# sair-lab/AirSLAM

Measured on AMD Instinct MI355X. Metric: stereo detect+match pairs/sec (2x PLNet @512x512 internal: points + lines, junctions on the left + LightGlue match), higher is better.
Workload: dtype fp16

## Files before the change

### airslam_amd/_lib.py

```python
from __future__ import annotations

import ctypes as C
import os

_HERE = os.path.dirname(os.path.abspath(__file__))
LIB_PATH = os.path.join(_HERE, "libairfe.so")


class Tuning(C.Structure):
    _fields_ = [(n, C.c_int) for n in (
        "fuse_lg_block", "gemm_small_max_m", "gemm8_min_m", "gemmr_min_m", "gemmr_wgs", "qkv_pair", "block_min_m", "lgb_tokens", "sg_kenc_gemm",
        "fold_qkv", "overlap_lines", "kf_graph", "kf_spec_rows", "fuse_dec", "assign_fused", "fold_out_proj", "desc_gather_stream", "copy_wgs")] + [("reserved", C.c_int * 5)]


class Cfg(C.Structure):
    _fields_ = [
        ("device", C.c_int), ("precision", C.c_int), ("max_batch", C.c_int), ("enc_chunk", C.c_int),
        ("max_keypoints", C.c_int), ("keypoint_threshold", C.c_float), ("remove_borders", C.c_int),
        ("nms_radius", C.c_int), ("line_threshold", C.c_float), ("line_length_threshold", C.c_float),
        ("matcher", C.c_int), ("image_width", C.c_int), ("image_height", C.c_int), ("sinkhorn_iters", C.c_int),
        ("superpoint_pack", C.c_char_p), ("plnet_s1_pack", C.c_char_p), ("lightglue_pack", C.c_char_p),
        ("superglue_pack", C.c_char_p), ("matcher_precision", C.c_int), ("line_precision", C.c_int), ("check_launches", C.c_int),
        ("tuning", C.POINTER(Tuning)),
    ]


class Stage0(C.Structure):
# ... 224 lines not shown
```

### airslam_amd/api.py

```python
from __future__ import annotations

import ctypes as C
import os
import tempfile
from typing import Dict, Optional

import numpy as np

from . import _lib, weights as W

FEAT = 259


def _pack_arg(x, tmpfiles) -> Optional[bytes]:
    if x is None:
        return None
    if isinstance(x, (str, bytes, os.PathLike)):
        return os.fsencode(x)
    f = tempfile.NamedTemporaryFile(suffix=".airfe", delete=False)
    f.close()
    W.save_pack(f.name, x)
    tmpfiles.append(f.name)
    return f.name.encode()

# ... 485 lines not shown
    def debug_lg_block(self, attn, x32, w1, b1, w2, b2, prec, gamma=None, beta=None, wo=None, bo=None, relu=False, tokens_per_wg=128, mixed=False,
                       nqk=None, nv=None, rot=None, Np=0):
        f32 = lambda t: None if t is None else np.ascontiguousarray(t, np.float32)
        m = attn.shape[0]
        attn, w1, b1, w2, b2, gamma, beta, wo, bo = map(f32, (attn, w1, b1, w2, b2, gamma, beta, wo, bo))
        x32 = np.array(x32, np.float32, copy=True)
        xb = np.empty_like(x32)
        ptr = lambda t: None if t is None else t.ctypes.data
        a = _lib.DebugLgBlockArgs(prec=prec, M=m, attn=ptr(attn), x32=ptr(x32), xb=ptr(xb), wo=ptr(wo), bo=ptr(bo), w1=ptr(w1), b1=ptr(b1), gamma=ptr(gamma),
                                  beta=ptr(beta), w2=ptr(w2), b2=ptr(b2), relu=int(relu), tokens_per_wg=tokens_per_wg, mixed=int(mixed), Np=Np)
        q = k = vt = None
        keep = []
        if nqk is not None:
            (qw, qb), (vw, vb) = map(lambda p: (f32(p[0]), f32(p[1])), (nqk, nv))
            keep += [qw, qb, vw, vb]
            s = m // Np
            q, vt = np.empty((s, 4, Np, 64), np.float32), np.empty((s, 4, 64, Np), np.float32)
            a.nqk_n, a.nqk_w, a.nqk_b, a.nv_w, a.nv_b, a.q, a.vt = qw.shape[0], ptr(qw), ptr(qb), ptr(vw), ptr(vb), ptr(q), ptr(vt)
            if qw.shape[0] == 512:
                k = np.empty_like(q)
                a.k = ptr(k)
        if rot is not None:
            rc, rs = f32(rot[0]), f32(rot[1])
            keep += [rc, rs]
            a.rot_cos, a.rot_sin = ptr(rc), ptr(rs)
        self._chk(self._l.airfe_debug_lg_block(self._h, C.byref(a)), "airfe_debug_lg_block")
        return {"x32": x32, "xb": xb, "q": q, "k": k, "vt": vt, "rows_past": list(a.rows_past)}

    def debug_ln_gelu(self, h, gamma, beta, prec):
        h = np.array(h, np.float32, copy=True)
        gamma, beta = np.ascontiguousarray(gamma, np.float32), np.ascontiguousarray(beta, np.float32)
# ... 476 lines not shown
```

### airslam_amd/csrc/airfe.hip

```cpp
#include "airfe_host.h"
#include "fransac_core.h"
#include "pnp_core.h"
#include "poseopt_core.h"
#include "bowgroup_core.h"

namespace airfe_host {
thread_local std::string g_err;

int fail(airfe_ctx* c, const std::string& m) {
  if (c) c->err = m;
  g_err = m;
  return 1;
}

int fail_noexcept(airfe_ctx* c, const char* what, const char* detail) noexcept {
  try {
    std::string m = std::string("airfe: C++ exception at the C boundary (") + what + "): " + (detail ? detail : "unknown");
    if (c) c->err = m;
    g_err = m;
  } catch (...) {
  }
  return 1;
}

// ... 184 lines not shown
    if (t->block_min_m >= 0) c->block_min = t->block_min_m;
    if (t->lgb_tokens >= 0) {
      if (t->lgb_tokens != 32 && t->lgb_tokens != 64 && t->lgb_tokens != 112 && t->lgb_tokens != 128) { return fail(nullptr, "airfe_create: tuning.lgb_tokens must be 32, 64, 112 or 128"); }
      c->lgb_tokens = t->lgb_tokens;
    }
    if (t->sg_kenc_gemm >= 0) c->sg_kenc_gemm = t->sg_kenc_gemm != 0;
    if (t->fold_qkv >= 0) c->fold_qkv = t->fold_qkv != 0;
    if (t->overlap_lines >= 0) c->overlap_lines = t->overlap_lines != 0;
    if (t->kf_graph >= 0) c->kf_graph_on = t->kf_graph != 0;
    if (t->kf_spec_rows >= 0) c->kf_spec_lines = c->kf_spec_juncs = std::max(t->kf_spec_rows, 1);
    if (t->fuse_dec >= 0) c->fuse_dec = t->fuse_dec != 0;
    if (t->assign_fused >= 0) c->assign_fused = t->assign_fused != 0 ? 1 : 0;
    if (t->fold_out_proj >= 0) c->fold_out = t->fold_out_proj != 0;
    if (t->desc_gather_stream >= 0) c->desc_gather_stream = t->desc_gather_stream != 0;
    if (t->copy_wgs > 0) c->copy_wgs = t->copy_wgs;
  }
  if (hipStreamCreateWithFlags(&c->stream, hipStreamNonBlocking) != hipSuccess ||
      hipStreamCreateWithFlags(&c->stream2, hipStreamNonBlocking) != hipSuccess ||
      hipEventCreateWithFlags(&c->ev_fork, hipEventDisableTiming) != hipSuccess ||
      hipEventCreateWithFlags(&c->ev_join, hipEventDisableTiming) != hipSuccess ||
      hipEventCreateWithFlags(&c->ev_feat, hipEventDisableTiming) != hipSuccess)
    return fail(nullptr, "airfe_create: stream creation failed");
  c->Dmax = (c->prec != 2 && cfg->superpoint_pack && cfg->lightglue_pack) ? 2 * c->Bmax : c->Bmax;
  c->chunk = std::min(std::max(cfg->enc_chunk, 1), c->Dmax);
  c->Lmax = c->Dmax;
  int rc = 0;
  if (cfg->superpoint_pack) rc = load_superpoint(c, cfg->superpoint_pack);
  if (!rc && cfg->lightglue_pack) rc = load_lightglue(c, cfg->lightglue_pack);
  if (!rc && cfg->superglue_pack) rc = load_superglue(c, cfg->superglue_pack);
  if (!rc && cfg->plnet_s1_pack) rc = load_plnet_s1(c, cfg->plnet_s1_pack);
// ... 1763 lines not shown
  return rc;
} AIRFE_CATCH(c)

int airfe_debug_lg_block(airfe_ctx* c, airfe_debug_lg_block_args* a) try {
  AIRFE_ENTER(c);
  if (!a || !a->attn || !a->x32 || !a->xb || !a->w1 || !a->b1 || !a->w2 || !a->b2 || (!a->relu && (!a->gamma || !a->beta)) || (!a->wo) != (!a->bo))
    return fail(c, "debug_lg_block: null argument");
  const int prec = a->prec, M = a->M, T = a->tokens_per_wg, nq = a->nqk_n, Np = a->Np;
  if ((prec != 0 && prec != 1) || M < 1 || (T != 32 && T != 64 && T != 112 && T != 128) || (nq != 0 && nq != 256 && nq != 512) || (a->relu && nq))
    return fail(c, "debug_lg_block: bad argument");
  if (a->mixed) {
    const int tiles = (M + 15) / 16, W = c->n_cu;
    if (a->wo || T != 112 || W <= 0 || tiles <= 7 * W || tiles > 13 * W) return fail(c, "debug_lg_block: the mixed split does not apply to this form");
  }
  if (nq && (!a->nqk_w || !a->nqk_b || !a->nv_w || !a->nv_b || !a->q || !a->vt || (nq == 512) != (a->rot_cos && a->rot_sin) || (nq == 512 && !a->k) || Np < 16 ||
             Np % 16 || M % Np))
    return fail(c, "debug_lg_block: the next projection needs its weights and outputs, rotary exactly when nqk_n = 512, and M = S * Np (Np a multiple of 16)");
  const int cap = M + 256;
  const int Sg = nq ? (cap + Np - 1) / Np : 0, S = nq ? M / Np : 0;
  const size_t helems = (size_t)Sg * 4 * Np * 64;
  airfe_ctx tmp;
  tmp.prec = prec;
  tmp.pack_prec = prec;
  LinW lo, l1, l2, lq, lv;
  bool ok = (!a->wo || make_linear(&tmp, a->wo, a->bo, 256, 256, lo)) && make_linear(&tmp, a->w1, a->b1, 512, 512, l1) && make_linear(&tmp, a->w2, a->b2, 512, 256, l2) &&
            (!nq || (make_linear(&tmp, a->nqk_w, a->nqk_b, 256, nq, lq) && make_linear(&tmp, a->nv_w, a->nv_b, 256, 256, lv)));
  const bool fr = lg_blockf_frag_weights();
  std::vector<float> x32h = dbg_rows4(a->x32, M, 256, cap);
  std::vector<uint16_t> xbh((size_t)cap * 256);
  for (size_t i = 0; i < xbh.size(); ++i) xbh[i] = cvt2(x32h[i], prec);
  std::vector<float> gb(1024, 0.f);
  if (!a->relu) { memcpy(gb.data(), a->gamma, 512 * 4); memcpy(gb.data() + 512, a->beta, 512 * 4); }
  LgBlockFArgs g;
  g.attn = dupload(&tmp, dbg_rows2(a->attn, M, 256, cap, prec));
  g.xb = dupload(&tmp, xbh);
  g.x32 = dupload(&tmp, x32h);
  const float* dgb = dupload(&tmp, gb);
  g.wo = a->wo ? (fr ? lo.wf : lo.w) : nullptr; g.bo = a->wo ? lo.b : nullptr;
  g.w1 = fr ? l1.wf : l1.w; g.b1 = l1.b; g.w2 = fr ? l2.wf : l2.w; g.b2 = l2.b;
  g.gamma = dgb; g.beta = dgb ? dgb + 512 : nullptr;
  g.M = M; g.tokens_per_wg = T; g.mixed = a->mixed; g.n_cu = c->n_cu; g.relu = a->relu;
  if (nq) {
    g.nqk_w = fr ? lq.wf : lq.w; g.nqk_b = lq.b; g.nqk_n = nq; g.nv_w = fr ? lv.wf : lv.w; g.nv_b = lv.b; g.Np = Np; g.H = 4;
    if (nq == 512) { g.rot_cos = dupload(&tmp, dbg_rows4(a->rot_cos, M, 32, cap)); g.rot_sin = dupload(&tmp, dbg_rows4(a->rot_sin, M, 32, cap)); }
    g.q_out = dbg_canary<uint16_t>(&tmp, helems);
    if (nq == 512) g.k_out = dbg_canary<uint16_t>(&tmp, helems);
    g.vt_out = dbg_canary<uint16_t>(&tmp, helems);
  }
  ok = ok && g.attn && g.xb && g.x32 && dgb && (!nq || (g.q_out && g.vt_out && (nq != 512 || (g.k_out && g.rot_cos && g.rot_sin))));
  int rc = ok ? 0 : fail(c, "debug_lg_block: allocation failed");
  if (!rc) {
    launch_lg_blockf(prec, g, c->stream);
    if (hipStreamSynchronize(c->stream) != hipSuccess || launch_status(c)) rc = fail(c, "debug_lg_block: kernel failed");
  }
  if (!rc) {
    std::vector<float> x32o((size_t)cap * 256);
// ... 5 lines not shown
    for (int i = 0; i < 5; ++i) a->rows_past[i] = 0;
    for (int r = M; r < cap; ++r)
      for (int f = 0; f < 256; ++f) {
        const size_t e = (size_t)r * 256 + f;
        if (memcmp(&x32o[e], &x32h[e], 4)) a->rows_past[0] = r - M + 1;
        if (xbo[e] != xbh[e]) a->rows_past[1] = r - M + 1;
      }
    if (nq) {
      uint16_t* dev[3] = {g.q_out, g.k_out, g.vt_out};
      float* host[3] = {a->q, a->k, a->vt};
      std::vector<uint16_t> ho(helems);
      for (int j = 0; j < 3; ++j) {
        if (!dev[j]) continue;
        (void)hipMemcpy(ho.data(), dev[j], helems * 2, hipMemcpyDeviceToHost);
        dbg_back2(ho, (size_t)S * 4 * Np * 64, prec, host[j]);
        for (size_t e = (size_t)S * 4 * Np * 64; e < helems; ++e) {
          if (ho[e] == 0xFFFF) continue;
          const size_t s = e / ((size_t)4 * Np * 64), w = e % ((size_t)Np * 64);
          const int row = (int)(s * Np + (j == 2 ? w % Np : w / 64));
          a->rows_past[2 + j] = std::max(a->rows_past[2 + j], row - M + 1);
        }
      }
    }
  }
  for (void* p : tmp.allocs) (void)hipFree(p);
  return rc;
} AIRFE_CATCH(c)

int airfe_debug_ln_gelu(airfe_ctx* c, int prec, float* h, const float* gamma, const float* beta, int M) try {
  AIRFE_ENTER(c);
  if ((prec != 0 && prec != 1) || M < 1 || !h || !gamma || !beta) return fail(c, "debug_ln_gelu: bad argument");
  airfe_ctx tmp;
  std::vector<float> gb(1024);
  memcpy(gb.data(), gamma, 512 * 4);
// ... 689 lines not shown
```

### airslam_amd/csrc/airfe_host.h

```cpp
#pragma once
#include "../../include/airfe.h"
#include "../../include/airfe_debug.h"

#include <hip/hip_runtime.h>

#include <algorithm>
#include <cmath>
#include <cstdio>
#include <cstdlib>
#include <cstring>
#include <functional>
#include <map>
#include <string>
#include <vector>

#include "kernels.h"
#include "common.h"

using namespace airfe;


namespace airfe_host {

extern thread_local std::string g_err;
// ... 50 lines not shown
  void* copy_ring = nullptr;
  int copy_ring_cap = 0, copy_ring_slot = 0, copy_wgs = 64;
  int *sat_host = nullptr, *sat_flag = nullptr;
  bool fuse_dec = true;
  int assign_fused = 0;
  hipStream_t stream = nullptr;
  hipStream_t stream2 = nullptr;
  hipEvent_t ev_fork = nullptr, ev_join = nullptr, ev_feat = nullptr;
  bool overlap_lines = true;
  std::vector<void*> allocs;
  int prec = 0;
  int mprec = 1;
  int pack_prec = 0;
  int Bmax = 1, chunk = 1, Np = 64, Pmax = 1;
  int lgb_tokens = 0;
  uint8_t* pin = nullptr;
  size_t pin_bytes = 0;
  uint8_t *io_in = nullptr, *io_out = nullptr;
  bool trace_overflow = false;
  size_t arena_rows = 0;
  int Dmax = 1;
  bool has_sp = false, has_lg = false;
  uint8_t* pl_stage = nullptr;
  size_t pl_bytes = 0;
  uint8_t *pl_scratch = nullptr, *ml_scratch = nullptr;
  size_t pl_scratch_bytes = 0, ml_scratch_bytes = 0;
  hipStream_t pl_scratch_stream = nullptr, ml_scratch_stream = nullptr;
  uint8_t* fr_scratch = nullptr; size_t fr_scratch_bytes = 0;
  hipStream_t fr_scratch_stream = nullptr;
  uint8_t* fr_stage = nullptr; size_t fr_stage_bytes = 0;
// ... 247 lines not shown
```

### airslam_amd/csrc/airfe_match.hip

```cpp
#include "airfe_host.h"

namespace airfe_host {

int lightglue_dev_f32(airfe_ctx* c, const float* f0, const int* n0, const float* f1, const int* n1, int B, int cap, int ld, int kp_off,
                      int normalize, int32_t* d_idx, float* d_score, int mcap, int* d_nmatch, float* scores_out, hipStream_t st) {
  const int S = 2 * B, Np = c->Np, M = S * Np;
  LgPrepArgs pa;
  pa.f0 = f0; pa.f1 = f1; pa.n0 = n0; pa.n1 = n1; pa.ld = ld; pa.kp_off = kp_off; pa.normalize = normalize;
  pa.cx = (float)(c->cfg.image_width / 2);
  pa.cy = (float)(c->cfg.image_height / 2);
  pa.linv = (float)(1.0 / std::max(c->cfg.image_width, c->cfg.image_height) * (double)0.5f);
  pa.wr = c->lg_wr; pa.B = B; pa.cap = cap; pa.Np = Np;
  pa.x32 = c->x32; pa.xb = c->xb; pa.rot_cos = c->rot_cos; pa.rot_sin = c->rot_sin; pa.lens = c->lens;
  pa.slack_rows = (int)(c->arena_rows - (size_t)M);
  launch_lg_prepare(1, pa, st);
  auto lin = [&](const airfe_ctx::F32Lin& w, const float* x1, int ld1, int K1, const float* x2, int ld2, float* y, int ldy, int acc, float scale = 1.f) {
    GemmF32Args g;
    g.X1 = x1; g.ld1 = ld1; g.K1 = K1; g.X2 = x2; g.ld2 = ld2; g.W = w.w; g.bias = w.b; g.Y = y; g.ldy = ldy;
    g.M = M; g.N = w.N; g.K = w.K; g.accumulate = acc; g.scale = scale;
    launch_gemm_f32(g, st);
  };
  auto ffn = [&](const airfe_ctx::F32Lin& f0w, const float* g, const float* b, const airfe_ctx::F32Lin& f3w) {
    lin(f0w, c->x32, 256, 256, c->m_msg, 256, c->m_h, 512, 0);
    launch_ln_gelu_f32(c->m_h, g, b, M, st);
// ... 123 lines not shown

int lg_blockf(airfe_ctx* c, const LinW& out, const LinW& f0, const float* g, const float* b, const LinW& f3, int M, hipStream_t st, int relu = 0,
               const LinW* nqk = nullptr, const LinW* nv = nullptr, bool rotary = false) {
  LgBlockFArgs a;
  a.relu = relu;
  const bool fr = lg_blockf_frag_weights();
  a.attn = c->ob; a.xb = c->xb; a.x32 = c->x32; a.wo = fr ? out.wf : out.w; a.w1 = fr ? f0.wf : f0.w; a.w2 = fr ? f3.wf : f3.w;
  a.bo = out.b; a.b1 = f0.b; a.gamma = g; a.beta = b; a.b2 = f3.b; a.M = M;
  if (c->fold_out) { a.wo = nullptr; a.bo = nullptr; }
  a.tokens_per_wg = ((M + 111) / 112 + 255) / 256 * 112 < ((M + 127) / 128 + 255) / 256 * 128 ? 112 : 128;
  if (M <= 256 * 32) a.tokens_per_wg = 32;
  else if (M <= 256 * 64) a.tokens_per_wg = 64;
  if (c->lgb_tokens > 0) a.tokens_per_wg = c->lgb_tokens;
  a.mixed = c->lgb_tokens <= 0;
  a.n_cu = c->n_cu;
  double fl = 2.0 * M * ((c->fold_out ? 0.0 : 256.0 * 256) + 512.0 * 512 + 512.0 * 256), by = (double)M * (512 + 512 + 1024 + 512 + 1024) + (c->fold_out ? 786432.0 : 917504.0);
  if (nqk && nv) {
    a.nqk_w = fr ? nqk->wf : nqk->w; a.nqk_b = nqk->b; a.nqk_n = nqk->N; a.nv_w = fr ? nv->wf : nv->w; a.nv_b = nv->b;
    a.rot_cos = rotary ? c->rot_cos : nullptr; a.rot_sin = rotary ? c->rot_sin : nullptr;
    a.q_out = c->qb; a.k_out = c->kb; a.vt_out = c->vtb; a.Np = c->Np; a.H = 4;
    fl += 2.0 * M * 256.0 * (nqk->N + nv->N);
    by += (double)M * (nqk->N + nv->N) * 2 + 256.0 * (nqk->N + nv->N) * 2;
  }
  { ProfScope ps(c, ST_LG_GEMM, st, fl, by); launch_lg_blockf(c->mprec, a, st); }
  return STAGE_RC(c);
}

int lg_ffn(airfe_ctx* c, const LinW& f0, const float* g, const float* b, const LinW& f3, int M, hipStream_t st) {
  RUN(run_linear(c, f0, c->xb, 256, 256, c->fold_out ? c->ob : c->msg, 256, M, EPI_STORE, ACT_NONE, c->hb, 512, st));
  { ProfScope ps(c, ST_LG_LNGELU, st, 0, (double)M * 2048); launch_ln_gelu(c->mprec, c->hb, g, b, M, st); }
// ... 194 lines not shown
```

### airslam_amd/csrc/kernels.h

```cpp
#pragma once
#include <hip/hip_runtime.h>
#include <stdint.h>

namespace airfe {

enum Epi {
  EPI_STORE = 0,
  EPI_STORE_F32 = 1,
  EPI_RESID = 2,
  EPI_HEADS = 3,
  EPI_HEADS_T = 4,
  EPI_SOFTMAX_D2S = 5
};
enum Act { ACT_NONE = 0, ACT_RELU = 1 };

struct GemmArgs {
  const uint16_t* X1 = nullptr;
  const uint16_t* X2 = nullptr;
  int ld1 = 0, ld2 = 0, K1 = 0;
  const uint16_t* Wp = nullptr;
  const float* bias = nullptr;
  int M = 0;
  int N = 0;
  int cb_total = 0;
// ... 23 lines not shown
bool gemmr_gather128_applicable(const GemmArgs& a);
void launch_gemmr_gather128(int prec, const GemmArgs& a, hipStream_t st);
bool gemmr_pair_applicable(const GemmArgs& a, const GemmArgs& b);
void launch_gemmr_pair(int prec, const GemmArgs& a, const GemmArgs& b, hipStream_t st);

struct LgBlockFArgs {
  const uint16_t* attn;
  uint16_t* xb;
  float* x32;
  const uint16_t *wo, *w1, *w2;
  const float *bo, *b1, *gamma, *beta, *b2;
  int M;
  int tokens_per_wg = 128;
  int mixed = 0, n_cu = 0;
  int relu = 0;
  const uint16_t *nqk_w = nullptr, *nv_w = nullptr;
  const float *nqk_b = nullptr, *nv_b = nullptr, *rot_cos = nullptr, *rot_sin = nullptr;
  int nqk_n = 0, Np = 0, H = 4;
  uint16_t *q_out = nullptr, *k_out = nullptr, *vt_out = nullptr;
};
void launch_lg_blockf(int prec, const LgBlockFArgs& a, hipStream_t st);
bool lg_blockf_frag_weights();

struct ConvArgs {
  const uint16_t* X = nullptr;
  const uint16_t* Wp = nullptr;
  const float* bias = nullptr;
  uint16_t* Y = nullptr;
  int B = 0, H = 0, W = 0, CIN = 0, COUT = 0;
  int pool = 0;
// ... 306 lines not shown
```

### airslam_amd/csrc/kernels_lgblockf.hip

```cpp
#include "common.h"
#include "kernels.h"
#ifdef LF_TIMING
__device__ unsigned long long lf_dbg[32];
#define LF_T(i) { const long long now_ = wall_clock64(); if (L.wave == 0 && L.lane == 0) atomicAdd(&lf_dbg[L.tb + i], (unsigned long long)(now_ - tp_)); tp_ = now_; }
extern "C" void airfe_dbg_lf(unsigned long long* out, int reset) {
  if (reset) { unsigned long long z[32] = {}; (void)hipMemcpyToSymbol(HIP_SYMBOL(lf_dbg), z, sizeof(z)); }
  else (void)hipMemcpyFromSymbol(out, HIP_SYMBOL(lf_dbg), 32 * sizeof(unsigned long long));
}
#else
#define LF_T(i)
#endif
#ifdef LF_TIMING2
__device__ unsigned long long lf2_dbg[16];
extern "C" void airfe_dbg_lf2(unsigned long long* out, int reset) {
  if (reset) { unsigned long long z[16] = {}; (void)hipMemcpyToSymbol(HIP_SYMBOL(lf2_dbg), z, sizeof(z)); }
  else (void)hipMemcpyFromSymbol(out, HIP_SYMBOL(lf2_dbg), 16 * sizeof(unsigned long long));
}
#define LF2_NOW(v) { __builtin_amdgcn_sched_barrier(0); v = __builtin_readcyclecounter(); __builtin_amdgcn_sched_barrier(0); }
#endif

namespace airfe {

constexpr int LF_R0 = 0, LF_R1 = 65536, LF_ST = 131072;
constexpr int LF_LDS = LF_ST + 8 * 128 * 8;

#ifndef LF_FRAG
#define LF_FRAG 1
#endif
constexpr int LF_SS = LF_FRAG ? 2048 : SLAB_BYTES;
constexpr int lf_ts(int K) { return LF_FRAG ? (K / 64) * 2048 : 2048; }
constexpr int LF_TS256 = lf_ts(256), LF_TS512 = lf_ts(512);
__device__ __forceinline__ size_t lf_woff(int K, int cb, int t0) {
  return LF_FRAG ? (size_t)(cb * 4 + t0) * (K / 64) * 2048 : (size_t)cb * (K / 64) * SLAB_BYTES + (size_t)t0 * 2048;
}

__device__ __forceinline__ void lf_glds16(const void* gsrc, unsigned lds_off) {
  unsigned keep;
  asm volatile("s_mov_b32 %0, m0\n\ts_mov_b32 m0, %2\n\ts_nop 0\n\tglobal_load_lds_dwordx4 %1, off\n\ts_mov_b32 m0, %0"
               : "=&s"(keep)
// ... 74 lines not shown
__device__ __forceinline__ void lf_first(typename P::vec8 (&cur)[NT][2], const char* w0, const char* w1) {
#pragma unroll
  for (int t = 0; t < NT; ++t) {
    cur[t][0] = lf_ldg<P>(w0 + t * TS);
    cur[t][1] = lf_ldg<P>(w1 + t * TS);
  }
}

struct LfNoHook { __device__ __forceinline__ void operator()(int) const {} };

#ifndef LF_GELU_X4
#define LF_GELU_X4 1
#endif


template <class P, int NT, int NMT, int TS, int TSN, class Hook = LfNoHook, bool SWAP = false, bool TIMED = false>
__device__ __forceinline__ void lf_mma(f32x4 (&acc)[NT][NMT], typename P::vec8 (&cur)[NT][2], const char* w0, const char* w1, int nslab,
                                       const char* n0, const char* n1, const char* breg, int pitch, int l15, int g, Hook hook = Hook()) {
  const char* brow = breg + l15 * pitch;
  if constexpr (NMT <= 4) {
    typename P::vec8 ring[8][NT][2];
    auto fetch = [&](int k, typename P::vec8 (&dst)[NT][2]) {
      const char* p0 = k == nslab ? n0 : w0 + k * LF_SS;
      const char* p1 = k == nslab ? n1 : w1 + k * LF_SS;
      const int ts = k == nslab ? TSN : TS;
#pragma unroll
      for (int t = 0; t < NT; ++t) {
        dst[t][0] = lf_ldg<P>(p0 + t * ts);
        dst[t][1] = lf_ldg<P>(p1 + t * ts);
      }
// ... 145 lines not shown
      atomicAdd(&lf2_dbg[5], a_mov); atomicAdd(&lf2_dbg[6], a_trips); atomicAdd(&lf2_dbg[7], (unsigned long long)(2 * ((NMT + 3) / 4)) * a_trips);
      atomicAdd(&lf2_dbg[8], (unsigned long long)(2 * NT * NMT) * a_trips);
    }
  }
#endif
}

struct LfLane {
  int lane, wave, l15, g, wf, cb, tp, fo0, fo1;
#ifdef LF_TIMING
  int tb;
#endif
  const char *wob, *w1b, *w2b;
};

template <class P, int NMT, bool RELU, int FOLD, bool FOLDO>
__device__ __forceinline__ void lf_pass(const LgBlockFArgs& a, char* smem, const LfLane& L, int row0) {
  const int lane = L.lane, wave = L.wave, l15 = L.l15, g = L.g, wf = L.wf, cb = L.cb, tp = L.tp, fo0 = L.fo0, fo1 = L.fo1;
#ifdef LF_TIMING
  long long tp_ = wall_clock64();
  if (wave == 0 && lane == 0) atomicAdd(&lf_dbg[L.tb + 15], 1ull);
#endif
  typename P::vec8 c2[2][2], c4[4][2];
  [[maybe_unused]] f32x4 bo2[2];
  f32x4 b14[4];
  if constexpr (FOLDO) {
    lf_first<P, 4, LF_TS512>(c4, L.w1b + 4 * LF_SS + fo0, L.w1b + 4 * LF_SS + fo1);
  } else {
    lf_first<P, 2, LF_TS256>(c2, L.wob + fo0, L.wob + fo1);
#pragma unroll
    for (int u = 0; u < 2; ++u) bo2[u] = *reinterpret_cast<const f32x4*>(a.bo + cb * 64 + tp * 32 + g * 8 + u * 4);
  }
// ... 165 lines not shown
#pragma unroll
        for (int m = 0; m < NMT; ++m) {
          r0[m] = *reinterpret_cast<const float4*>(xr0 + (size_t)m * 16 * 256);
          r1[m] = *reinterpret_cast<const float4*>(xr0 + (size_t)m * 16 * 256 + 4);
        }
        __builtin_amdgcn_sched_barrier(0);
      }
    }
  }
  if constexpr (!EARLY_W2) lf_first<P, 2, LF_TS512>(c2, L.w2b + fo0, L.w2b + fo1);
  LF_T(6)
  __syncthreads();
  LF_T(7)

  constexpr bool KEEP_X = FOLD != 0 && NMT < 8;
  [[maybe_unused]] uint4 xpk[KEEP_X ? NMT : 1];
  {
    f32x4 acc[2][NMT];
#pragma unroll
    for (int u = 0; u < 2; ++u)
#pragma unroll
      for (int m = 0; m < NMT; ++m) acc[u][m] = b22[u];
    const char* nq = FOLD ? reinterpret_cast<const char*>(a.nqk_w) + lf_woff(256, cb, 2 * tp) : L.w2b;
    lf_mma<P, 2, NMT, LF_TS512, (FOLD ? LF_TS256 : LF_TS512)>(acc, c2, L.w2b + fo0, L.w2b + fo1, 8, nq + fo0, nq + fo1, smem, 1024, l15, g);
#pragma unroll
    for (int m = 0; m < NMT; ++m) {
      const size_t row = (size_t)(row0 + m * 16 + l15);
      float* xr = xr0 + (size_t)m * 16 * 256;
      float v[8] = {acc[0][m][0] + r0[m].x, acc[0][m][1] + r0[m].y, acc[0][m][2] + r0[m].z, acc[0][m][3] + r0[m].w,
                    acc[1][m][0] + r1[m].x, acc[1][m][1] + r1[m].y, acc[1][m][2] + r1[m].z, acc[1][m][3] + r1[m].w};
      *reinterpret_cast<float4*>(xr) = make_float4(v[0], v[1], v[2], v[3]);
      *reinterpret_cast<float4*>(xr + 4) = make_float4(v[4], v[5], v[6], v[7]);
      const uint4 xp = pack8<P>(v);
      if constexpr (KEEP_X) xpk[m] = xp;
      *reinterpret_cast<uint4*>(a.xb + row * 256 + co) = xp;
    }
  }
  LF_T(8)
  if constexpr (FOLD != 0) {
    __syncthreads();
    {
      const int piece = cb * 8 + tp * 4 + g;
#pragma unroll
      for (int m = 0; m < NMT; ++m) {
        uint4 xp;
        if constexpr (KEEP_X) xp = xpk[m];
        else xp = *reinterpret_cast<const uint4*>(a.xb + (size_t)(row0 + m * 16 + l15) * 256 + co);
        *reinterpret_cast<uint4*>(smem + LF_R0 + (m * 16 + l15) * 512 + ((piece ^ l15) << 4)) = xp;
      }
    }
    __syncthreads();
    LF_T(9)
    const int H = a.H, Np = a.Np;
    constexpr int NQ = FOLD == 2 ? 2 : 1;
    const char* vbase = reinterpret_cast<const char*>(a.nv_w) + lf_woff(256, cb, 2 * tp);
#pragma unroll
    for (int qu = 0; qu < NQ; ++qu) {
      const int cbq = cb + 4 * qu;
      const char* wq = reinterpret_cast<const char*>(a.nqk_w) + lf_woff(256, cbq, 2 * tp);
      const char* nx = (qu + 1 < NQ) ? reinterpret_cast<const char*>(a.nqk_w) + lf_woff(256, cbq + 4, 2 * tp) : vbase;
      const int cq = cbq * 64 + tp * 32 + g * 8;
      f32x4 bq[2];
#pragma unroll
      for (int u = 0; u < 2; ++u) bq[u] = *reinterpret_cast<const f32x4*>(a.nqk_b + cq + u * 4);
      f32x4 acc[2][NMT];
#pragma unroll
      for (int u = 0; u < 2; ++u)
#pragma unroll
// ... 32 lines not shown
      lf_mma<P, 2, NMT, LF_TS256, LF_TS256, LfNoHook, true>(acc, c2, vbase + fo0, vbase + fo1, 4, vbase + fo0, vbase + fo1, smem + LF_R0, 512, l15, g);
#pragma unroll
      for (int u = 0; u < 2; ++u) {
        const int cv = cb * 64 + slab_row_to_feature((2 * tp + u) * 16 + l15);
        const int hh = cv >> 6, d = cv & 63;
#pragma unroll
        for (int m = 0; m < NMT; ++m) {
          const int rw = row0 + m * 16 + g * 4;
          const int sq = rw / Np, nn = rw - sq * Np;
          *reinterpret_cast<uint2*>(a.vt_out + (((size_t)sq * H + hh) * 64 + d) * Np + nn) =
                pack4<P>(acc[u][m][0] + bt[u], acc[u][m][1] + bt[u], acc[u][m][2] + bt[u], acc[u][m][3] + bt[u]);
        }
      }
    }
    LF_T(11)
  }
}

__device__ __forceinline__ void lf_lane_init(const LgBlockFArgs& a, LfLane& L) {
  const int tid = threadIdx.x;
  L.lane = tid & 63;
  L.wave = __builtin_amdgcn_readfirstlane(tid >> 6);
  L.l15 = L.lane & 15;
  L.g = L.lane >> 4;
  if (LF_FRAG) {
    L.fo0 = L.lane * 16;
    L.fo1 = L.lane * 16 + 1024;
  } else {
    const int sw = (L.l15 >> 1) & 7;
    L.fo0 = L.l15 * 128 + ((L.g ^ sw) << 4);
    L.fo1 = L.l15 * 128 + (((4 + L.g) ^ sw) << 4);
  }
  L.wf = (L.wave + (blockIdx.x >> 3)) & 7;
  L.cb = L.wf >> 1;
  L.tp = L.wf & 1;
  L.wob = reinterpret_cast<const char*>(a.wo) + lf_woff(256, L.cb, 2 * L.tp);
  L.w1b = reinterpret_cast<const char*>(a.w1) + lf_woff(512, L.wf, 0);
  L.w2b = reinterpret_cast<const char*>(a.w2) + lf_woff(512, L.cb, 2 * L.tp);
}

template <class P, int NMT, bool RELU, int FOLD, bool FOLDO>
__global__ __launch_bounds__(512, 1) void lg_blockf_kernel(LgBlockFArgs a) {
  extern __shared__ __attribute__((aligned(16))) char smem[];
  LfLane L;
  lf_lane_init(a, L);
  const int row0 = blockIdx.x * (16 * NMT);
  lf_stage_rows(a.attn, row0, NMT, FOLDO ? LF_R1 : LF_R0, L.wave, L.lane);
  if constexpr (FOLDO) lf_stage_rows(a.xb, row0, NMT, LF_R0, L.wave, L.lane);
#ifdef LF_TIMING
  L.tb = 0;
#endif
  lf_pass<P, NMT, RELU, FOLD, FOLDO>(a, smem, L, row0);
#ifdef LF_TWICE
  __syncthreads();
  L.tb = 16;
  lf_stage_rows(a.attn, row0, NMT, FOLDO ? LF_R1 : LF_R0, L.wave, L.lane);
  if constexpr (FOLDO) lf_stage_rows(a.xb, row0, NMT, LF_R0, L.wave, L.lane);
  lf_pass<P, NMT, RELU, FOLD, FOLDO>(a, smem, L, row0);
#endif
}

template <class P, bool RELU, int FOLD>
__global__ __launch_bounds__(512, 1) void lg_blockf_mixed_kernel(LgBlockFArgs a, int n7) {
  extern __shared__ __attribute__((aligned(16))) char smem[];
  LfLane L;
  lf_lane_init(a, L);
#ifdef LF_TIMING
  L.tb = 0;
#endif
  if ((int)blockIdx.x < n7) {
    const int row0 = blockIdx.x * 112;
    lf_stage_rows(a.attn, row0, 7, LF_R1, L.wave, L.lane);
    lf_stage_rows(a.xb, row0, 7, LF_R0, L.wave, L.lane);
    lf_pass<P, 7, RELU, FOLD, true>(a, smem, L, row0);
  } else {
    const int row0 = n7 * 112 + ((int)blockIdx.x - n7) * 96;
    lf_stage_rows(a.attn, row0, 6, LF_R1, L.wave, L.lane);
    lf_stage_rows(a.xb, row0, 6, LF_R0, L.wave, L.lane);
    lf_pass<P, 6, RELU, FOLD, true>(a, smem, L, row0);
  }
}

template <class P, bool RELU, int FOLD>
static bool launch_mixed(const LgBlockFArgs& a, hipStream_t st) {
  const int tiles = (a.M + 15) / 16, W = a.n_cu;
  if (!a.mixed || a.wo || W <= 0 || tiles <= 7 * W || tiles > 13 * W) return false;
  const int n7 = W, n6 = (tiles - 7 * W + 5) / 6;
  static PerDeviceOnce attr_once;
  auto kfn = lg_blockf_mixed_kernel<P, RELU, FOLD>;
  if (auto once_token = attr_once.first()) {
    (void)hipFuncSetAttribute(reinterpret_cast<const void*>(kfn), hipFuncAttributeMaxDynamicSharedMemorySize, LF_LDS);
  }
  hipLaunchKernelGGL(kfn, dim3((unsigned)(n7 + n6)), dim3(512), LF_LDS, st, a, n7);
  return true;
}

template <class P, int NMT, bool RELU, int FOLD, bool FOLDO>
static void launch_fo(const LgBlockFArgs& a, hipStream_t st) {
  static PerDeviceOnce attr_once;
  auto kfn = lg_blockf_kernel<P, NMT, RELU, FOLD, FOLDO>;
  if (auto once_token = attr_once.first()) {
    (void)hipFuncSetAttribute(reinterpret_cast<const void*>(kfn), hipFuncAttributeMaxDynamicSharedMemorySize, LF_LDS);
  }
  hipLaunchKernelGGL(kfn, dim3((unsigned)((a.M + 16 * NMT - 1) / (16 * NMT))), dim3(512), LF_LDS, st, a);
}

template <class P, int NMT, bool RELU, int FOLD = 0>
static void launch_f(const LgBlockFArgs& a, hipStream_t st) {
  if (a.wo) launch_fo<P, NMT, RELU, FOLD, false>(a, st);
  else launch_fo<P, NMT, RELU, FOLD, true>(a, st);
}

template <class P, bool RELU, int FOLD>
static void launch_nmt(const LgBlockFArgs& a, hipStream_t st) {
  switch (a.tokens_per_wg) {
    case 32: launch_f<P, 2, RELU, FOLD>(a, st); break;
    case 64: launch_f<P, 4, RELU, FOLD>(a, st); break;
    case 112: if (!launch_mixed<P, RELU, FOLD>(a, st)) launch_f<P, 7, RELU, FOLD>(a, st); break;
    default: launch_f<P, 8, RELU, FOLD>(a, st); break;
// ... 23 lines not shown
```

### include/airfe.h

```cpp
#ifndef AIRFE_H_
#define AIRFE_H_

#include <stddef.h>
#include <stdint.h>

#ifdef __cplusplus
extern "C" {
#endif

#define AIRFE_FEAT_DIM 259
#define AIRFE_INTERNAL_SIZE 512

typedef struct airfe_ctx airfe_ctx;

typedef struct airfe_tuning {
  int fuse_lg_block;
  int gemm_small_max_m;
  int gemm8_min_m;
  int gemmr_min_m;
  int gemmr_wgs;
  int qkv_pair;
  int block_min_m;
  int lgb_tokens;
  int sg_kenc_gemm;
  int fold_qkv;
  int overlap_lines;
  int kf_graph;
  int kf_spec_rows;
  int fuse_dec;
  int assign_fused;
  int fold_out_proj;
  int desc_gather_stream;
  int copy_wgs;
  int reserved[5];
} airfe_tuning;

typedef struct airfe_cfg {
  int device;
  int precision;
  int max_batch;
  int enc_chunk;
  int max_keypoints;
  float keypoint_threshold;
  int remove_borders;
  int nms_radius;
  float line_threshold;
  float line_length_threshold;
  int matcher;
  int image_width;
// ... 193 lines not shown
```

Before: 7967.

## Overlap folded QKV projection epilogues with next projection's MFMA loop

Adds an epilogue-overlap mode to the fused LightGlue block kernel. The folded Q/K/V projections are restructured so that each projection's bias, rotary and store epilogue, plus the rotary-table loads, are interleaved via hooks into the next projection's MFMA slab loop, instead of running serially after it. Mode 2 also defers the residual x stores into the first projection's loop. This is meant to hide global load and store latency behind matrix work, at the cost of higher register pressure and more template instantiations. Mode 1 is on by default.

```diff
diff --git a/airslam_amd/_lib.py b/airslam_amd/_lib.py
--- a/airslam_amd/_lib.py
+++ b/airslam_amd/_lib.py
@@ -11,6 +11,14 @@
     _fields_ = [(n, C.c_int) for n in (
         "fuse_lg_block", "gemm_small_max_m", "gemm8_min_m", "gemmr_min_m", "gemmr_wgs", "qkv_pair", "block_min_m", "lgb_tokens", "sg_kenc_gemm",
         "fold_qkv", "overlap_lines", "kf_graph", "kf_spec_rows", "fuse_dec", "assign_fused", "fold_out_proj", "desc_gather_stream", "copy_wgs")] + [("reserved", C.c_int * 5)]
+
+    @property
+    def lgb_epi_overlap(self):
+        return self.reserved[0]
+
+    @lgb_epi_overlap.setter
+    def lgb_epi_overlap(self, v):
+        self.reserved[0] = int(v)
 
 
 class Cfg(C.Structure):
diff --git a/airslam_amd/api.py b/airslam_amd/api.py
--- a/airslam_amd/api.py
+++ b/airslam_amd/api.py
@@ -523,7 +523,7 @@
         if nqk is not None:
             (qw, qb), (vw, vb) = map(lambda p: (f32(p[0]), f32(p[1])), (nqk, nv))
             keep += [qw, qb, vw, vb]
-            s = m // Np
+            s = -(-m // Np)
             q, vt = np.empty((s, 4, Np, 64), np.float32), np.empty((s, 4, 64, Np), np.float32)
             a.nqk_n, a.nqk_w, a.nqk_b, a.nv_w, a.nv_b, a.q, a.vt = qw.shape[0], ptr(qw), ptr(qb), ptr(vw), ptr(vb), ptr(q), ptr(vt)
             if qw.shape[0] == 512:
diff --git a/airslam_amd/csrc/airfe.hip b/airslam_amd/csrc/airfe.hip
--- a/airslam_amd/csrc/airfe.hip
+++ b/airslam_amd/csrc/airfe.hip
@@ -222,6 +222,10 @@
     if (t->fold_out_proj >= 0) c->fold_out = t->fold_out_proj != 0;
     if (t->desc_gather_stream >= 0) c->desc_gather_stream = t->desc_gather_stream != 0;
     if (t->copy_wgs > 0) c->copy_wgs = t->copy_wgs;
+    if (t->lgb_epi_overlap >= 0) {
+      if (t->lgb_epi_overlap > 2) { return fail(nullptr, "airfe_create: tuning.lgb_epi_overlap must be 0, 1 or 2"); }
+      c->lgb_epi_overlap = t->lgb_epi_overlap;
+    }
   }
   if (hipStreamCreateWithFlags(&c->stream, hipStreamNonBlocking) != hipSuccess ||
       hipStreamCreateWithFlags(&c->stream2, hipStreamNonBlocking) != hipSuccess ||
@@ -2015,10 +2019,10 @@
     if (a->wo || T != 112 || W <= 0 || tiles <= 7 * W || tiles > 13 * W) return fail(c, "debug_lg_block: the mixed split does not apply to this form");
   }
   if (nq && (!a->nqk_w || !a->nqk_b || !a->nv_w || !a->nv_b || !a->q || !a->vt || (nq == 512) != (a->rot_cos && a->rot_sin) || (nq == 512 && !a->k) || Np < 16 ||
-             Np % 16 || M % Np))
-    return fail(c, "debug_lg_block: the next projection needs its weights and outputs, rotary exactly when nqk_n = 512, and M = S * Np (Np a multiple of 16)");
+             Np % 16))
+    return fail(c, "debug_lg_block: the next projection needs its weights and outputs, rotary exactly when nqk_n = 512, and Np a multiple of 16");
   const int cap = M + 256;
-  const int Sg = nq ? (cap + Np - 1) / Np : 0, S = nq ? M / Np : 0;
+  const int Sg = nq ? (cap + Np - 1) / Np : 0, S = nq ? (M + Np - 1) / Np : 0, Sfull = nq ? M / Np : 0;
   const size_t helems = (size_t)Sg * 4 * Np * 64;
   airfe_ctx tmp;
   tmp.prec = prec;
@@ -2040,7 +2044,7 @@
   g.wo = a->wo ? (fr ? lo.wf : lo.w) : nullptr; g.bo = a->wo ? lo.b : nullptr;
   g.w1 = fr ? l1.wf : l1.w; g.b1 = l1.b; g.w2 = fr ? l2.wf : l2.w; g.b2 = l2.b;
   g.gamma = dgb; g.beta = dgb ? dgb + 512 : nullptr;
-  g.M = M; g.tokens_per_wg = T; g.mixed = a->mixed; g.n_cu = c->n_cu; g.relu = a->relu;
+  g.M = M; g.tokens_per_wg = T; g.mixed = a->mixed; g.n_cu = c->n_cu; g.relu = a->relu; g.epi_overlap = c->lgb_epi_overlap;
   if (nq) {
     g.nqk_w = fr ? lq.wf : lq.w; g.nqk_b = lq.b; g.nqk_n = nq; g.nv_w = fr ? lv.wf : lv.w; g.nv_b = lv.b; g.Np = Np; g.H = 4;
     if (nq == 512) { g.rot_cos = dupload(&tmp, dbg_rows4(a->rot_cos, M, 32, cap)); g.rot_sin = dupload(&tmp, dbg_rows4(a->rot_sin, M, 32, cap)); }
@@ -2076,10 +2080,11 @@
         if (!dev[j]) continue;
         (void)hipMemcpy(ho.data(), dev[j], helems * 2, hipMemcpyDeviceToHost);
         dbg_back2(ho, (size_t)S * 4 * Np * 64, prec, host[j]);
-        for (size_t e = (size_t)S * 4 * Np * 64; e < helems; ++e) {
+        for (size_t e = (size_t)Sfull * 4 * Np * 64; e < helems; ++e) {
           if (ho[e] == 0xFFFF) continue;
           const size_t s = e / ((size_t)4 * Np * 64), w = e % ((size_t)Np * 64);
           const int row = (int)(s * Np + (j == 2 ? w % Np : w / 64));
+          if (row < M) continue;
           a->rows_past[2 + j] = std::max(a->rows_past[2 + j], row - M + 1);
         }
       }
diff --git a/airslam_amd/csrc/airfe_host.h b/airslam_amd/csrc/airfe_host.h
--- a/airslam_amd/csrc/airfe_host.h
+++ b/airslam_amd/csrc/airfe_host.h
@@ -88,6 +88,7 @@
   int pack_prec = 0;
   int Bmax = 1, chunk = 1, Np = 64, Pmax = 1;
   int lgb_tokens = 0;
+  int lgb_epi_overlap = 1;
   uint8_t* pin = nullptr;
   size_t pin_bytes = 0;
   uint8_t *io_in = nullptr, *io_out = nullptr;
diff --git a/airslam_amd/csrc/airfe_match.hip b/airslam_amd/csrc/airfe_match.hip
--- a/airslam_amd/csrc/airfe_match.hip
+++ b/airslam_amd/csrc/airfe_match.hip
@@ -161,6 +161,7 @@
   if (c->lgb_tokens > 0) a.tokens_per_wg = c->lgb_tokens;
   a.mixed = c->lgb_tokens <= 0;
   a.n_cu = c->n_cu;
+  a.epi_overlap = c->lgb_epi_overlap;
   double fl = 2.0 * M * ((c->fold_out ? 0.0 : 256.0 * 256) + 512.0 * 512 + 512.0 * 256), by = (double)M * (512 + 512 + 1024 + 512 + 1024) + (c->fold_out ? 786432.0 : 917504.0);
   if (nqk && nv) {
     a.nqk_w = fr ? nqk->wf : nqk->w; a.nqk_b = nqk->b; a.nqk_n = nqk->N; a.nv_w = fr ? nv->wf : nv->w; a.nv_b = nv->b;
diff --git a/airslam_amd/csrc/kernels.h b/airslam_amd/csrc/kernels.h
--- a/airslam_amd/csrc/kernels.h
+++ b/airslam_amd/csrc/kernels.h
@@ -61,6 +61,7 @@
   int tokens_per_wg = 128;
   int mixed = 0, n_cu = 0;
   int relu = 0;
+  int epi_overlap = 0;
   const uint16_t *nqk_w = nullptr, *nv_w = nullptr;
   const float *nqk_b = nullptr, *nv_b = nullptr, *rot_cos = nullptr, *rot_sin = nullptr;
   int nqk_n = 0, Np = 0, H = 4;
diff --git a/airslam_amd/csrc/kernels_lgblockf.hip b/airslam_amd/csrc/kernels_lgblockf.hip
--- a/airslam_amd/csrc/kernels_lgblockf.hip
+++ b/airslam_amd/csrc/kernels_lgblockf.hip
@@ -1,5 +1,6 @@
 #include "common.h"
 #include "kernels.h"
+#include <utility>
 #ifdef LF_TIMING
 __device__ unsigned long long lf_dbg[32];
 #define LF_T(i) { const long long now_ = wall_clock64(); if (L.wave == 0 && L.lane == 0) atomicAdd(&lf_dbg[L.tb + i], (unsigned long long)(now_ - tp_)); tp_ = now_; }
@@ -23,6 +24,7 @@
 
 constexpr int LF_R0 = 0, LF_R1 = 65536, LF_ST = 131072;
 constexpr int LF_LDS = LF_ST + 8 * 128 * 8;
+static_assert(LF_LDS == 139264, "136 KiB: R0 + R1 + the LayerNorm sums; every instantiation is launched with exactly this");
 
 #ifndef LF_FRAG
 #define LF_FRAG 1
@@ -127,6 +129,69 @@
 #endif
 
 
+template <int... I, class F>
+__device__ __forceinline__ void lf_seq(std::integer_sequence<int, I...>, F&& f) { (f(std::integral_constant<int, I>{}), ...); }
+template <int N, class F>
+__device__ __forceinline__ void lf_static_for(F&& f) { lf_seq(std::make_integer_sequence<int, N>{}, f); }
+
+template <class P, int NMT, bool SWAP, class Hook>
+__device__ __forceinline__ void lf_mma4(f32x4 (&acc)[2][NMT], typename P::vec8 (&cur)[2][2], const char* w0, const char* w1, const char* n0, const char* n1,
+                                        const char* breg, int l15, int g, Hook hook) {
+  constexpr int NT = 2, pitch = 512, DEPTH = NMT <= 4 ? 4 : 1;
+  const char* brow = breg + l15 * pitch;
+  asm volatile("" ::: "memory");
+  typename P::vec8 ring[DEPTH][NT][2];
+  auto fetch = [&](int k, typename P::vec8 (&dst)[NT][2]) {
+    const char* p0 = k == 4 ? n0 : w0 + k * LF_SS;
+    const char* p1 = k == 4 ? n1 : w1 + k * LF_SS;
+#pragma unroll
+    for (int t = 0; t < NT; ++t) {
+      dst[t][0] = lf_ldg<P>(p0 + t * LF_TS256);
+      dst[t][1] = lf_ldg<P>(p1 + t * LF_TS256);
+    }
+  };
+  if constexpr (DEPTH == 4) {
+#pragma unroll
+    for (int d = 0; d < 4; ++d) fetch(d + 1, ring[d]);
+    __builtin_amdgcn_sched_barrier(0);
+  }
+  lf_static_for<4>([&](auto sc) {
+    constexpr int s = decltype(sc)::value;
+    if constexpr (DEPTH == 1) fetch(s + 1, ring[0]);
+    hook(sc);
+    __builtin_amdgcn_sched_barrier(0);
+#pragma unroll
+    for (int h = 0; h < 2; ++h) {
+      const int boff = (((s * 8 + h * 4 + g) ^ l15) << 4);
+#pragma unroll
+      for (int mb = 0; mb < NMT; mb += 4) {
+        typename P::vec8 bf[4];
+#pragma unroll
+        for (int j = 0; j < 4; ++j)
+          if (mb + j < NMT) bf[j] = lds_frag<P>(brow, boff + (mb + j) * 16 * pitch);
+#pragma unroll
+        for (int t = 0; t < NT; ++t)
+#pragma unroll
+          for (int j = 0; j < 4; ++j)
+            if (mb + j < NMT) {
+              if constexpr (SWAP) acc[t][mb + j] = P::mfma(bf[j], cur[t][h], acc[t][mb + j]);
+              else acc[t][mb + j] = P::mfma(cur[t][h], bf[j], acc[t][mb + j]);
+            }
+      }
+    }
+#pragma unroll
+    for (int t = 0; t < NT; ++t) {
+      cur[t][0] = ring[DEPTH == 1 ? 0 : s][t][0];
+      cur[t][1] = ring[DEPTH == 1 ? 0 : s][t][1];
+    }
+#pragma unroll
+    for (int t = 0; t < NT; ++t)
+#pragma unroll
+      for (int m = 0; m < NMT; ++m) asm volatile("" : "+v"(acc[t][m]));
+    if constexpr (DEPTH == 4) __builtin_amdgcn_sched_barrier(0);
+  });
+}
+
 template <class P, int NT, int NMT, int TS, int TSN, class Hook = LfNoHook, bool SWAP = false, bool TIMED = false>
 __device__ __forceinline__ void lf_mma(f32x4 (&acc)[NT][NMT], typename P::vec8 (&cur)[NT][2], const char* w0, const char* w1, int nslab,
                                        const char* n0, const char* n1, const char* breg, int pitch, int l15, int g, Hook hook = Hook()) {
@@ -302,8 +367,9 @@
   const char *wob, *w1b, *w2b;
 };
 
-template <class P, int NMT, bool RELU, int FOLD, bool FOLDO>
+template <class P, int NMT, bool RELU, int FOLD, bool FOLDO, int EPI = 0>
 __device__ __forceinline__ void lf_pass(const LgBlockFArgs& a, char* smem, const LfLane& L, int row0) {
+  static_assert(EPI == 0 || FOLD != 0, "lgb_epi_overlap reorders the folded projections only");
   const int lane = L.lane, wave = L.wave, l15 = L.l15, g = L.g, wf = L.wf, cb = L.cb, tp = L.tp, fo0 = L.fo0, fo1 = L.fo1;
 #ifdef LF_TIMING
   long long tp_ = wall_clock64();
@@ -499,7 +565,9 @@
   LF_T(7)
 
   constexpr bool KEEP_X = FOLD != 0 && NMT < 8;
+  constexpr bool DEFER_X = KEEP_X && EPI >= 2;
   [[maybe_unused]] uint4 xpk[KEEP_X ? NMT : 1];
+  [[maybe_unused]] float xv[DEFER_X ? NMT : 1][8];
   {
     f32x4 acc[2][NMT];
 #pragma unroll
@@ -514,11 +582,16 @@
       float* xr = xr0 + (size_t)m * 16 * 256;
       float v[8] = {acc[0][m][0] + r0[m].x, acc[0][m][1] + r0[m].y, acc[0][m][2] + r0[m].z, acc[0][m][3] + r0[m].w,
                     acc[1][m][0] + r1[m].x, acc[1][m][1] + r1[m].y, acc[1][m][2] + r1[m].z, acc[1][m][3] + r1[m].w};
-      *reinterpret_cast<float4*>(xr) = make_float4(v[0], v[1], v[2], v[3]);
-      *reinterpret_cast<float4*>(xr + 4) = make_float4(v[4], v[5], v[6], v[7]);
       const uint4 xp = pack8<P>(v);
       if constexpr (KEEP_X) xpk[m] = xp;
-      *reinterpret_cast<uint4*>(a.xb + row * 256 + co) = xp;
+      if constexpr (DEFER_X) {
+#pragma unroll
+        for (int e = 0; e < 8; ++e) xv[m][e] = v[e];
+      } else {
+        *reinterpret_cast<float4*>(xr) = make_float4(v[0], v[1], v[2], v[3]);
+        *reinterpret_cast<float4*>(xr + 4) = make_float4(v[4], v[5], v[6], v[7]);
+        *reinterpret_cast<uint4*>(a.xb + row * 256 + co) = xp;
+      }
     }
   }
   LF_T(8)
@@ -537,6 +610,7 @@
     __syncthreads();
     LF_T(9)
     const int H = a.H, Np = a.Np;
+    if constexpr (EPI == 0) {
     constexpr int NQ = FOLD == 2 ? 2 : 1;
     const char* vbase = reinterpret_cast<const char*>(a.nv_w) + lf_woff(256, cb, 2 * tp);
 #pragma unroll
@@ -599,6 +673,114 @@
       }
     }
     LF_T(11)
+    } else {
+    constexpr int NQ = FOLD == 2 ? 2 : 1;
+    constexpr int TPT = (NMT + 3) / 4;
+    const char* vbase = reinterpret_cast<const char*>(a.nv_w) + lf_woff(256, cb, 2 * tp);
+    [[maybe_unused]] f32x4 rc[2][TPT], rs[2][TPT];
+    auto rot_req = [&](auto sc) {
+      if constexpr (FOLD == 2) {
+        constexpr int s = decltype(sc)::value;
+        lf_static_for<TPT>([&](auto jc) {
+          constexpr int j = decltype(jc)::value, m = s * TPT + j;
+          if constexpr (m < NMT) {
+            const size_t ro = (size_t)(row0 + m * 16 + l15) * 32 + tp * 16 + g * 4;
+            rc[s & 1][j] = *reinterpret_cast<const f32x4*>(a.rot_cos + ro);
+            rs[s & 1][j] = *reinterpret_cast<const f32x4*>(a.rot_sin + ro);
+          }
+        });
+        __builtin_amdgcn_sched_barrier(0);
+      }
+    };
+    auto qk_epi = [&](const f32x4 (&acc)[2][NMT], const f32x4 (&bq)[2], int cq, auto sc) {
+      constexpr int s = decltype(sc)::value;
+      const int sel = cq >> 8, hh = (cq & 255) >> 6, d = cq & 63;
+      uint16_t* ob = sel ? a.k_out : a.q_out;
+      lf_static_for<TPT>([&](auto jc) {
+        constexpr int j = decltype(jc)::value, m = s * TPT + j;
+        if constexpr (m < NMT) {
+          const int row = row0 + m * 16 + l15;
+          float v[8];
+#pragma unroll
+          for (int e = 0; e < 4; ++e) {
+            v[e] = acc[0][m][e] + bq[0][e];
+            v[4 + e] = acc[1][m][e] + bq[1][e];
+          }
+          if constexpr (FOLD == 2) rotate_pairs(v, rc[s & 1][j], rs[s & 1][j]);
+          const int sq = row / Np, nn = row - sq * Np;
+          *reinterpret_cast<uint4*>(ob + (((size_t)sq * H + hh) * Np + nn) * 64 + d) = pack8<P>(v);
+        }
+      });
+    };
+    [[maybe_unused]] auto x_stores = [&](auto sc) {
+      constexpr int s = decltype(sc)::value;
+      lf_static_for<TPT>([&](auto jc) {
+        constexpr int j = decltype(jc)::value, m = s * TPT + j;
+        if constexpr (DEFER_X && m < NMT) {
+          float* xr = xr0 + (size_t)m * 16 * 256;
+          *reinterpret_cast<float4*>(xr) = make_float4(xv[m][0], xv[m][1], xv[m][2], xv[m][3]);
+          *reinterpret_cast<float4*>(xr + 4) = make_float4(xv[m][4], xv[m][5], xv[m][6], xv[m][7]);
+          *reinterpret_cast<uint4*>(a.xb + (size_t)(row0 + m * 16 + l15) * 256 + co) = xpk[m];
+        }
+      });
+    };
+    f32x4 accq[NQ][2][NMT], bq[NQ][2];
+    int cqs[NQ];
+    lf_static_for<NQ>([&](auto qc) {
+      constexpr int qu = decltype(qc)::value, pu = qu ? qu - 1 : 0;
+      const int cbq = cb + 4 * qu;
+      const char* wq = reinterpret_cast<const char*>(a.nqk_w) + lf_woff(256, cbq, 2 * tp);
+      const char* nx = (qu + 1 < NQ) ? reinterpret_cast<const char*>(a.nqk_w) + lf_woff(256, cbq + 4, 2 * tp) : vbase;
+      cqs[qu] = cbq * 64 + tp * 32 + g * 8;
+#pragma unroll
+      for (int u = 0; u < 2; ++u) bq[qu][u] = *reinterpret_cast<const f32x4*>(a.nqk_b + cqs[qu] + u * 4);
+#pragma unroll
+      for (int u = 0; u < 2; ++u)
+#pragma unroll
+        for (int m = 0; m < NMT; ++m) accq[qu][u][m] = f32x4{0.f, 0.f, 0.f, 0.f};
+      auto hook = [&](auto sc) {
+        constexpr int s = decltype(sc)::value;
+        if constexpr (qu == 0) {
+          if constexpr (DEFER_X) x_stores(sc);
+          if constexpr (s == 3) rot_req(std::integral_constant<int, 0>{});
+        } else {
+          rot_req(std::integral_constant<int, (s + 1) & 3>{});
+          qk_epi(accq[pu], bq[pu], cqs[pu], sc);
+        }
+      };
+      lf_mma4<P, NMT, false>(accq[qu], c2, wq + fo0, wq + fo1, nx + fo0, nx + fo1, smem + LF_R0, l15, g, hook);
+    });
+    LF_T(10)
+    {
+      float bt[2];
+#pragma unroll
+      for (int u = 0; u < 2; ++u) bt[u] = a.nv_b[cb * 64 + slab_row_to_feature((2 * tp + u) * 16 + l15)];
+      f32x4 acc[2][NMT];
+#pragma unroll
+      for (int u = 0; u < 2; ++u)
+#pragma unroll
+        for (int m = 0; m < NMT; ++m) acc[u][m] = f32x4{0.f, 0.f, 0.f, 0.f};
+      auto hook = [&](auto sc) {
+        constexpr int s = decltype(sc)::value;
+        if constexpr (s < 3) rot_req(std::integral_constant<int, s + 1>{});
+        qk_epi(accq[NQ - 1], bq[NQ - 1], cqs[NQ - 1], sc);
+      };
+      lf_mma4<P, NMT, true>(acc, c2, vbase + fo0, vbase + fo1, vbase + fo0, vbase + fo1, smem + LF_R0, l15, g, hook);
+#pragma unroll
+      for (int u = 0; u < 2; ++u) {
+        const int cv = cb * 64 + slab_row_to_feature((2 * tp + u) * 16 + l15);
+        const int hh = cv >> 6, d = cv & 63;
+#pragma unroll
+        for (int m = 0; m < NMT; ++m) {
+          const int rw = row0 + m * 16 + g * 4;
+          const int sq = rw / Np, nn = rw - sq * Np;
+          *reinterpret_cast<uint2*>(a.vt_out + (((size_t)sq * H + hh) * 64 + d) * Np + nn) =
+                pack4<P>(acc[u][m][0] + bt[u], acc[u][m][1] + bt[u], acc[u][m][2] + bt[u], acc[u][m][3] + bt[u]);
+        }
+      }
+    }
+    LF_T(11)
+    }
   }
 }
 
@@ -624,7 +806,7 @@
   L.w2b = reinterpret_cast<const char*>(a.w2) + lf_woff(512, L.cb, 2 * L.tp);
 }
 
-template <class P, int NMT, bool RELU, int FOLD, bool FOLDO>
+template <class P, int NMT, bool RELU, int FOLD, bool FOLDO, int EPI>
 __global__ __launch_bounds__(512, 1) void lg_blockf_kernel(LgBlockFArgs a) {
   extern __shared__ __attribute__((aligned(16))) char smem[];
   LfLane L;
@@ -635,17 +817,17 @@
 #ifdef LF_TIMING
   L.tb = 0;
 #endif
-  lf_pass<P, NMT, RELU, FOLD, FOLDO>(a, smem, L, row0);
+  lf_pass<P, NMT, RELU, FOLD, FOLDO, EPI>(a, smem, L, row0);
 #ifdef LF_TWICE
   __syncthreads();
   L.tb = 16;
   lf_stage_rows(a.attn, row0, NMT, FOLDO ? LF_R1 : LF_R0, L.wave, L.lane);
   if constexpr (FOLDO) lf_stage_rows(a.xb, row0, NMT, LF_R0, L.wave, L.lane);
-  lf_pass<P, NMT, RELU, FOLD, FOLDO>(a, smem, L, row0);
-#endif
-}
-
-template <class P, bool RELU, int FOLD>
+  lf_pass<P, NMT, RELU, FOLD, FOLDO, EPI>(a, smem, L, row0);
+#endif
+}
+
+template <class P, bool RELU, int FOLD, int EPI>
 __global__ __launch_bounds__(512, 1) void lg_blockf_mixed_kernel(LgBlockFArgs a, int n7) {
   extern __shared__ __attribute__((aligned(16))) char smem[];
   LfLane L;
@@ -657,13 +839,26 @@
     const int row0 = blockIdx.x * 112;
     lf_stage_rows(a.attn, row0, 7, LF_R1, L.wave, L.lane);
     lf_stage_rows(a.xb, row0, 7, LF_R0, L.wave, L.lane);
-    lf_pass<P, 7, RELU, FOLD, true>(a, smem, L, row0);
+    lf_pass<P, 7, RELU, FOLD, true, EPI>(a, smem, L, row0);
   } else {
     const int row0 = n7 * 112 + ((int)blockIdx.x - n7) * 96;
     lf_stage_rows(a.attn, row0, 6, LF_R1, L.wave, L.lane);
     lf_stage_rows(a.xb, row0, 6, LF_R0, L.wave, L.lane);
-    lf_pass<P, 6, RELU, FOLD, true>(a, smem, L, row0);
-  }
+    lf_pass<P, 6, RELU, FOLD, true, EPI>(a, smem, L, row0);
+  }
+}
+
+template <int FOLD, int NMT>
+constexpr int lf_epi_max() { return FOLD == 0 || NMT >= 8 ? 0 : 2; }
+
+template <class P, bool RELU, int FOLD, int EPI>
+static void launch_mixed_e(const LgBlockFArgs& a, hipStream_t st, int n7, int n6) {
+  static PerDeviceOnce attr_once;
+  auto kfn = lg_blockf_mixed_kernel<P, RELU, FOLD, EPI>;
+  if (auto once_token = attr_once.first()) {
+    (void)hipFuncSetAttribute(reinterpret_cast<const void*>(kfn), hipFuncAttributeMaxDynamicSharedMemorySize, LF_LDS);
+  }
+  hipLaunchKernelGGL(kfn, dim3((unsigned)(n7 + n6)), dim3(512), LF_LDS, st, a, n7);
 }
 
 template <class P, bool RELU, int FOLD>
@@ -671,23 +866,31 @@
   const int tiles = (a.M + 15) / 16, W = a.n_cu;
   if (!a.mixed || a.wo || W <= 0 || tiles <= 7 * W || tiles > 13 * W) return false;
   const int n7 = W, n6 = (tiles - 7 * W + 5) / 6;
+  constexpr int EMAX = lf_epi_max<FOLD, 7>();
+  const int e = a.epi_overlap < EMAX ? a.epi_overlap : EMAX;
+  if constexpr (EMAX >= 2) { if (e == 2) { launch_mixed_e<P, RELU, FOLD, 2>(a, st, n7, n6); return true; } }
+  if constexpr (EMAX >= 1) { if (e == 1) { launch_mixed_e<P, RELU, FOLD, 1>(a, st, n7, n6); return true; } }
+  launch_mixed_e<P, RELU, FOLD, 0>(a, st, n7, n6);
+  return true;
+}
+
+template <class P, int NMT, bool RELU, int FOLD, bool FOLDO, int EPI>
+static void launch_fo_e(const LgBlockFArgs& a, hipStream_t st) {
   static PerDeviceOnce attr_once;
-  auto kfn = lg_blockf_mixed_kernel<P, RELU, FOLD>;
+  auto kfn = lg_blockf_kernel<P, NMT, RELU, FOLD, FOLDO, EPI>;
   if (auto once_token = attr_once.first()) {
     (void)hipFuncSetAttribute(reinterpret_cast<const void*>(kfn), hipFuncAttributeMaxDynamicSharedMemorySize, LF_LDS);
   }
-  hipLaunchKernelGGL(kfn, dim3((unsigned)(n7 + n6)), dim3(512), LF_LDS, st, a, n7);
-  return true;
+  hipLaunchKernelGGL(kfn, dim3((unsigned)((a.M + 16 * NMT - 1) / (16 * NMT))), dim3(512), LF_LDS, st, a);
 }
 
 template <class P, int NMT, bool RELU, int FOLD, bool FOLDO>
 static void launch_fo(const LgBlockFArgs& a, hipStream_t st) {
-  static PerDeviceOnce attr_once;
-  auto kfn = lg_blockf_kernel<P, NMT, RELU, FOLD, FOLDO>;
-  if (auto once_token = attr_once.first()) {
-    (void)hipFuncSetAttribute(reinterpret_cast<const void*>(kfn), hipFuncAttributeMaxDynamicSharedMemorySize, LF_LDS);
-  }
-  hipLaunchKernelGGL(kfn, dim3((unsigned)((a.M + 16 * NMT - 1) / (16 * NMT))), dim3(512), LF_LDS, st, a);
+  constexpr int EMAX = lf_epi_max<FOLD, NMT>();
+  const int e = a.epi_overlap < EMAX ? a.epi_overlap : EMAX;
+  if constexpr (EMAX >= 2) { if (e == 2) return launch_fo_e<P, NMT, RELU, FOLD, FOLDO, 2>(a, st); }
+  if constexpr (EMAX >= 1) { if (e == 1) return launch_fo_e<P, NMT, RELU, FOLD, FOLDO, 1>(a, st); }
+  launch_fo_e<P, NMT, RELU, FOLD, FOLDO, 0>(a, st);
 }
 
 template <class P, int NMT, bool RELU, int FOLD = 0>
diff --git a/include/airfe.h b/include/airfe.h
--- a/include/airfe.h
+++ b/include/airfe.h
@@ -32,7 +32,8 @@
   int fold_out_proj;
   int desc_gather_stream;
   int copy_wgs;
-  int reserved[5];
+  int lgb_epi_overlap;
+  int reserved[4];
 } airfe_tuning;
 
 typedef struct airfe_cfg {
```

After: 8008 (median of 6 runs). Within noise of the previous version (+0.5%).
